# frasermince/gym-cellular-automata

Hardware: AMD Instinct MI355X
Metric: cell-updates/sec, 4096x(256x256) ForestFireBulldozer (Alexandridis CA), per-GPU batch (higher is better)
Workload: dtype u8 cells / i16 ages / f32 probabilities

## Files before the change

gym-cellular-automata_amd/csrc/gca_alex_march.hip:

```cpp
#include "gca_alex_rule.h"

#include <type_traits>

#ifndef GCA_MARCH_FLAT_OCC
#define GCA_MARCH_FLAT_OCC 4
#endif
#ifndef GCA_MARCH_OBS_FLAT_OCC
#define GCA_MARCH_OBS_FLAT_OCC 3
#endif
#ifndef GCA_MARCH_XROW
#define GCA_MARCH_XROW 1
#endif

namespace {

constexpr int MW = 256;
constexpr int SH = 16;

struct MarchObs {
    const float4* col;
    const int32_t* night;
    float* rgb;
    const int32_t* action;
    int action_stride, n_choices;
    uint32_t mode_bits;
    uint8_t* refit;
};
constexpr uint32_t OBS_GRID = 0u, OBS_ZERO = 1u, OBS_NONE = 2u;
constexpr uint32_t OBS_CHK_GRID = 4u, OBS_CHK_BLUR = 8u;

__device__ __forceinline__ uint32_t from_prev(uint32_t v) {
    return (uint32_t)__builtin_amdgcn_mov_dpp((int)v, 0x138, 0xF, 0xF, true);
}
__device__ __forceinline__ uint32_t from_next(uint32_t v) {
    return (uint32_t)__builtin_amdgcn_mov_dpp((int)v, 0x130, 0xF, 0xF, true);
}
__device__ __forceinline__ uint32_t from_prev_or(uint32_t old, uint32_t v) {
    return (uint32_t)__builtin_amdgcn_update_dpp((int)old, (int)v, 0x138, 0xF, 0xF, false);
}
__device__ __forceinline__ uint32_t from_next_or(uint32_t old, uint32_t v) {
    return (uint32_t)__builtin_amdgcn_update_dpp((int)old, (int)v, 0x130, 0xF, 0xF, false);
}

template <int J> __device__ __forceinline__ uint64_t byte_lanes(uint32_t x) {
    static_assert(J >= 0 && J < 4, "byte 0..3");
    uint64_t m;
    const uint32_t zero = 0u;
    if constexpr (J == 0) asm("v_cmp_ne_u32_sdwa %0, %1, %2 src0_sel:BYTE_0 src1_sel:DWORD" : "=s"(m) : "v"(x), "s"(zero));
    if constexpr (J == 1) asm("v_cmp_ne_u32_sdwa %0, %1, %2 src0_sel:BYTE_1 src1_sel:DWORD" : "=s"(m) : "v"(x), "s"(zero));
    if constexpr (J == 2) asm("v_cmp_ne_u32_sdwa %0, %1, %2 src0_sel:BYTE_2 src1_sel:DWORD" : "=s"(m) : "v"(x), "s"(zero));
    if constexpr (J == 3) asm("v_cmp_ne_u32_sdwa %0, %1, %2 src0_sel:BYTE_3 src1_sel:DWORD" : "=s"(m) : "v"(x), "s"(zero));
    return m;
}
__device__ __forceinline__ uint32_t lanes_select(uint32_t c, uint64_t m) {
    uint32_t o;
    asm("v_cndmask_b32_e64 %0, 0, %1, %2" : "=v"(o) : "v"(c), "s"(m));
    return o;
}

__host__ __device__ constexpr uint32_t win_mask(int o, int j, int k) {
    uint32_t m = 0;
    for (int b = 0; b < 4; ++b) {
        const int c = 4 * o + b - j;
        if (c >= -k && c <= k) m |= 1u << (8 * b);
    }
    return m;
}
__host__ __device__ constexpr bool win_full(int o, int j, int k) { return j - k <= 4 * o && 4 * o + 3 <= j + k; }
template <bool HALO = false>
__device__ __forceinline__ void window4(uint32_t X, int k, uint32_t (&B)[4], uint32_t z = 0u, uint32_t h1 = 0u,
                                        uint32_t h2 = 0u) {
    uint32_t n[5] = {0u, 0u, X, 0u, 0u};
    if (k >= 1) {
        n[1] = HALO ? from_prev_or(h1, X) : from_prev(X);
        n[3] = HALO ? from_next_or(h1, X) : from_next(X);
    }
    if (k >= 5) {
        n[0] = HALO ? from_prev_or(h2, n[1]) : from_prev(n[1]);
        n[4] = HALO ? from_next_or(h2, n[3]) : from_next(n[3]);
    }
    constexpr uint32_t ONES = 0x01010101u;
    bool use0 = false, useL = false, useR = false, useLR = false;
#pragma unroll
    for (int j = 0; j < 4; ++j) {
        const bool f0 = win_full(0, j, k), fl = win_full(-1, j, k), fr = win_full(1, j, k);
        if (f0 && fl && fr) useLR = true;
        else if (f0 && fl) useL = true;
        else if (f0 && fr) useR = true;
        else if (f0) use0 = true;
    }
    uint32_t S0 = 0u, SL = 0u, SR = 0u, SLR = 0u;
    if (use0 || useL || useR || useLR) S0 = __builtin_amdgcn_udot4(n[2], ONES, z, false);
    if (useL || useLR) SL = __builtin_amdgcn_udot4(n[1], ONES, S0, false);
    if (useR) SR = __builtin_amdgcn_udot4(n[3], ONES, S0, false);
    if (useLR) SLR = __builtin_amdgcn_udot4(n[3], ONES, SL, false);
#pragma unroll
    for (int j = 0; j < 4; ++j) {
        const bool f0 = win_full(0, j, k), fl = win_full(-1, j, k), fr = win_full(1, j, k);
        const bool run = f0;
        uint32_t acc = !run ? z : (fl && fr) ? SLR : fl ? SL : fr ? SR : S0;
#pragma unroll
        for (int o = -2; o <= 2; ++o) {
            if (run && (o == 0 || (o == -1 && fl) || (o == 1 && fr))) continue;
            const uint32_t m = win_mask(o, j, k);
            if (m) acc = __builtin_amdgcn_udot4(n[o + 2], m, acc, false);
        }
        B[j] = acc;
    }
}

__device__ __forceinline__ float4 ldf4(const float* p) { return *reinterpret_cast<const float4*>(p); }
__device__ __forceinline__ gca_f2 m_recip(float v0, float v1) {
    const gca_f2 x = {v0, v1};
    const gca_f2 r0 = {__builtin_amdgcn_rcpf(v0), __builtin_amdgcn_rcpf(v1)};
    const gca_f2 ee = __builtin_elementwise_fma(-x, r0, (gca_f2){1.0f, 1.0f});
    return __builtin_elementwise_fma(ee, r0, r0);
}
__device__ __forceinline__ void m_edge_both(float v0, float v1, gca_f2& own, gca_f2& nb) {
    const gca_f2 rc = m_recip(v0, v1);
    asm("v_max_f32_e64 %0, %1, -%2" : "=v"(own.x) : "v"(v0), "v"(rc.x));
    asm("v_max_f32_e64 %0, %1, -%2" : "=v"(own.y) : "v"(v1), "v"(rc.y));
    asm("v_max_f32_e64 %0, -%1, %2" : "=v"(nb.x) : "v"(v0), "v"(rc.x));
    asm("v_max_f32_e64 %0, -%1, %2" : "=v"(nb.y) : "v"(v1), "v"(rc.y));
}
__device__ __forceinline__ void m_edge_both4(const float4& v, gca_f2& oa, gca_f2& na, gca_f2& ob, gca_f2& nb) {
    const gca_f2 x0 = {v.x, v.y}, x1 = {v.z, v.w};
    const gca_f2 r0 = {__builtin_amdgcn_rcpf(v.x), __builtin_amdgcn_rcpf(v.y)};
    const gca_f2 r1 = {__builtin_amdgcn_rcpf(v.z), __builtin_amdgcn_rcpf(v.w)};
    const gca_f2 e0 = __builtin_elementwise_fma(-x0, r0, (gca_f2){1.0f, 1.0f});
    const gca_f2 e1 = __builtin_elementwise_fma(-x1, r1, (gca_f2){1.0f, 1.0f});
    const gca_f2 c0 = __builtin_elementwise_fma(e0, r0, r0);
    const gca_f2 c1 = __builtin_elementwise_fma(e1, r1, r1);
    asm("v_max_f32_e64 %0, %1, -%2" : "=v"(oa.x) : "v"(v.x), "v"(c0.x));
    asm("v_max_f32_e64 %0, %1, -%2" : "=v"(oa.y) : "v"(v.y), "v"(c0.y));
    asm("v_max_f32_e64 %0, %1, -%2" : "=v"(ob.x) : "v"(v.z), "v"(c1.x));
    asm("v_max_f32_e64 %0, %1, -%2" : "=v"(ob.y) : "v"(v.w), "v"(c1.y));
    asm("v_max_f32_e64 %0, -%1, %2" : "=v"(na.x) : "v"(v.x), "v"(c0.x));
    asm("v_max_f32_e64 %0, -%1, %2" : "=v"(na.y) : "v"(v.y), "v"(c0.y));
    asm("v_max_f32_e64 %0, -%1, %2" : "=v"(nb.x) : "v"(v.z), "v"(c1.x));
    asm("v_max_f32_e64 %0, -%1, %2" : "=v"(nb.y) : "v"(v.w), "v"(c1.y));
}
__device__ __forceinline__ void m_edge_own4(const float4& v, gca_f2& oa, gca_f2& ob) {
    const gca_f2 x0 = {v.x, v.y}, x1 = {v.z, v.w};
    const gca_f2 r0 = {__builtin_amdgcn_rcpf(v.x), __builtin_amdgcn_rcpf(v.y)};
    const gca_f2 r1 = {__builtin_amdgcn_rcpf(v.z), __builtin_amdgcn_rcpf(v.w)};
    const gca_f2 e0 = __builtin_elementwise_fma(-x0, r0, (gca_f2){1.0f, 1.0f});
    const gca_f2 e1 = __builtin_elementwise_fma(-x1, r1, (gca_f2){1.0f, 1.0f});
    const gca_f2 c0 = __builtin_elementwise_fma(e0, r0, r0);
    const gca_f2 c1 = __builtin_elementwise_fma(e1, r1, r1);
    asm("v_max_f32_e64 %0, %1, -%2" : "=v"(oa.x) : "v"(v.x), "v"(c0.x));
    asm("v_max_f32_e64 %0, %1, -%2" : "=v"(oa.y) : "v"(v.y), "v"(c0.y));
    asm("v_max_f32_e64 %0, %1, -%2" : "=v"(ob.x) : "v"(v.z), "v"(c1.x));
    asm("v_max_f32_e64 %0, %1, -%2" : "=v"(ob.y) : "v"(v.w), "v"(c1.y));
}
template <class T, class B> __device__ __forceinline__ T ld_at(const B* base, uint32_t off) {
    return *reinterpret_cast<const T*>(reinterpret_cast<const unsigned char*>(base) + off);
}
template <class T, class B> __device__ __forceinline__ T ld_nt(const B* base, uint32_t off) {
    constexpr int N = (int)(sizeof(T) / 4);
    typedef uint32_t vt __attribute__((ext_vector_type(N)));
    typedef const __attribute__((address_space(1))) unsigned char gbyte;
    typedef const __attribute__((address_space(1))) vt gvt;
    const vt v = __builtin_nontemporal_load((gvt*)((gbyte*)base + off));
    return __builtin_bit_cast(T, v);
}
constexpr uint32_t WZ = 0x4B000000u;
__device__ __forceinline__ gca_f2 wsum_f2(uint32_t b0, uint32_t b1) {
    return (gca_f2){__uint_as_float(b0), __uint_as_float(b1)} - (gca_f2){8388608.0f, 8388608.0f};
}
typedef uint16_t u16x2 __attribute__((ext_vector_type(2)));
typedef int16_t i16x2 __attribute__((ext_vector_type(2)));
__device__ __forceinline__ i16x2 bitcast_i16x2(uint32_t v) { return __builtin_bit_cast(i16x2, v); }
__device__ __forceinline__ u16x2 bitcast_u16x2(uint32_t v) { return __builtin_bit_cast(u16x2, v); }
template <class T> __device__ __forceinline__ uint32_t bitcast_u32(T v) { return __builtin_bit_cast(uint32_t, v); }

constexpr int XI = 16;
constexpr int XS_ONE = 13, XS_TWO = 14;

template <int R, bool OBS, bool GROW, int NSEG, int FLATM>
__global__ __launch_bounds__(NSEG == 1 ? 256 : 64 * NSEG) __attribute__((amdgpu_waves_per_eu(OBS ? (FLATM ? GCA_MARCH_OBS_FLAT_OCC : 2) : (FLATM ? GCA_MARCH_FLAT_OCC : 3), OBS ? (FLATM ? GCA_MARCH_OBS_FLAT_OCC : 2) : (FLATM ? GCA_MARCH_FLAT_OCC : 3)))) void alex_march_kernel(
    gca_alex_params p, int H, int nwaves, const uint8_t* __restrict__ grid_in, uint8_t* __restrict__ grid_out,
    const int16_t* age_in, int16_t* age_out,
    const uint8_t* __restrict__ vd, const uint16_t* __restrict__ dbits, const float* __restrict__ es,
    const int32_t* __restrict__ wind_index, const uint32_t* __restrict__ rng_step, int32_t* __restrict__ counts,
    const uint8_t* __restrict__ act_in, uint8_t* __restrict__ act_out, MarchObs obs) {
    constexpr int NF = 2 * R + 1;
    constexpr int RB = R;
    constexpr bool HALO = NSEG > 1;
    constexpr bool SMASK = !HALO && !OBS && FLATM >= 1;
    constexpr int WPB = HALO ? NSEG : 4;
    constexpr int W = MW * NSEG;
    __shared__ float lut[WPB][16];
    __shared__ float4 colw[WPB][8];
    __shared__ float4 img[OBS ? WPB : 1][OBS ? 192 : 1];
    __shared__ uint32_t fring[WPB][2 * NF * 64];
    __shared__ uint32_t xch[HALO ? 2 : 1][HALO ? NSEG + 2 : 1][4][HALO ? XI : 1];
    __shared__ uint32_t qfl[HALO ? NSEG : 1];
    constexpr bool FLAT = FLATM >= 1, UNI = FLATM == 2;
    constexpr bool XROW = GCA_MARCH_XROW && !HALO && OBS && !FLAT;
    __shared__ float4 xrow[XROW ? 4 : 1][3][XROW ? 64 : 1];
    __shared__ uint32_t xok[XROW ? 4 : 1];

    const int tid = threadIdx.x, wl = __builtin_amdgcn_readfirstlane(tid >> 6), lane = tid & 63;
    const int nb = (int)gridDim.x;
    const int xcd = (int)blockIdx.x & 7, slot = (int)blockIdx.x >> 3;
    const int qn8 = nb >> 3, rn8 = nb & 7;
    const int lb = (xcd < rn8 ? xcd * (qn8 + 1) : rn8 * (qn8 + 1) + (xcd - rn8) * qn8) + slot;
    int strips, e, s, g;
    if constexpr (!HALO) {
        const int wv = lb * 4 + wl;
        if (wv >= nwaves) {
            if constexpr (XROW) {
                if (lane == 0) xok[wl] = 0u;
                __builtin_amdgcn_fence(__ATOMIC_RELEASE, "workgroup", "local");
                __builtin_amdgcn_s_barrier();
            }
            return;
        }
        strips = H / SH;
        e = wv / strips;
        s = wv - e * strips;
        g = 0;
    } else {
        if (lb * NSEG >= nwaves) return;
        strips = H / SH;
        e = lb / strips;
        s = lb - e * strips;
        g = wl;
    }
    const int s0 = s * SH;
    const uint32_t HW = (uint32_t)H * W;
    const uint8_t* gE = grid_in + (size_t)e * HW;
    uint8_t* gO = grid_out + (size_t)e * HW;
    const int16_t* aE = age_in + (size_t)e * HW;
    int16_t* aO = age_out + (size_t)e * HW;
    const uint8_t* vE = UNI ? vd : vd + (size_t)e * HW;
    const uint16_t* dE = dbits + (size_t)e * (HW >> 4);
    const float* sE = FLAT ? es : es + (size_t)e * 4 * HW;
    const uint32_t lc = HALO ? (uint32_t)(MW * g) + 4u * (uint32_t)lane : 4u * (uint32_t)lane;
    const uint32_t ld16 = HALO ? lc >> 4 : (uint32_t)(lane >> 2);
    const uint32_t lane_a = 2u * lc, lane_s = 4u * lc, lane_d = 2u * ld16;
    const uint32_t Fp = rep4((uint32_t)p.fire), Ep = rep4((uint32_t)p.empty), Tp = rep4((uint32_t)p.tree);

    if (lane < 16) lut[wl][lane] = gca_alex_lut_entry(p, lane);
    if (OBS && lane < 6) colw[wl][lane] = obs.col[6 * (obs.night[e] != 0 ? 1 : 0) + lane];
    uint32_t omode = 0u;
    if constexpr (OBS && !HALO) {
        if (obs.action) {
            const int choice = min(max(obs.action[(size_t)e * obs.action_stride + 2], 0), obs.n_choices - 1);
            omode = (uint32_t)__builtin_amdgcn_readfirstlane((int)((obs.mode_bits >> (4 * choice)) & 0xFu));
        }
    }
    auto row0_refit = [&](uint32_t x0, uint32_t x1) -> uint8_t {
        const uint32_t odd = ((x0 + 0x7D7D7D7Du) | x0 | (x1 + 0x7D7D7D7Du) | x1) & 0x80808080u;
        bool pos = false;
        if (omode & OBS_CHK_GRID) pos |= __ballot(x0 != 0u) != 0ull;
        if (omode & OBS_CHK_BLUR) {
            auto hsum = [&](uint32_t x) {
                uint32_t L = __builtin_amdgcn_alignbyte(x, from_prev(x), 3);
                uint32_t Rt = __builtin_amdgcn_alignbyte(from_next(x), x, 1);
                if (lane == 0) L = (x << 8) | (x & 0xFFu);
                if (lane == 63) Rt = (x >> 8) | (x & 0xFF000000u);
                return L + x + Rt;
            };
            const uint32_t S = 2u * hsum(x0) + hsum(x1);
            pos |= __ballot(((S + 0x7B7B7B7Bu) & 0x80808080u) != 0u) != 0ull;
        }
        const bool bad = __ballot(odd != 0u) != 0ull;
        return ((omode & 3u) == OBS_NONE || bad || ((omode & (OBS_CHK_GRID | OBS_CHK_BLUR)) && !pos)) ? 1 : 0;
    };
    __builtin_amdgcn_fence(__ATOMIC_RELEASE, "wavefront");
    __builtin_amdgcn_wave_barrier();
    __builtin_amdgcn_fence(__ATOMIC_ACQUIRE, "wavefront");

    auto graw = [&](int r) -> uint32_t {
        return (r >= 0 && r < H) ? *reinterpret_cast<const uint32_t*>(gE + (uint32_t)r * W + lc) : Ep;
    };
    auto draw_bits = [&](int r) -> uint32_t {
        return (r >= 0 && r < H) ? (uint32_t)dE[(uint32_t)r * (W / 16) + ld16] : 0u;
    };
    auto dflags = [&](uint32_t w16) -> uint32_t { return gca_spread4(w16 >> (4 * (lane & 3))); };
    auto write_rgb_row = [&](int r, uint32_t tB, uint32_t fB, uint32_t dfl) {
        if constexpr (OBS) {
            if ((omode & 3u) == OBS_NONE) return;
            if ((omode & 3u) == OBS_ZERO) tB = fB = 0u;
            const uint32_t kidx = 2u * gca_spread4(tB) + 4u * gca_spread4(fB) + (dfl & 0x01010101u);
            float* im = reinterpret_cast<float*>(img[wl]) + 12 * lane;
#pragma unroll
            for (int j = 0; j < 4; ++j) {
                const float4 c = colw[wl][(kidx >> (8 * j)) & 0xFFu];
                im[3 * j + 0] = c.x;
                im[3 * j + 1] = c.y;
                im[3 * j + 2] = c.z;
            }
            __builtin_amdgcn_fence(__ATOMIC_RELEASE, "wavefront");
            __builtin_amdgcn_wave_barrier();
            __builtin_amdgcn_fence(__ATOMIC_ACQUIRE, "wavefront");
            typedef float f4t __attribute__((ext_vector_type(4)));
            float* row = obs.rgb + ((size_t)e * H + r) * (W * 3) + (HALO ? (size_t)(MW * 3) * g : 0);
            float4 v[3];
#pragma unroll
            for (int t = 0; t < 3; ++t) v[t] = img[wl][64 * t + lane];
#pragma unroll
            for (int t = 0; t < 3; ++t)
                __builtin_nontemporal_store((f4t){v[t].x, v[t].y, v[t].z, v[t].w},
                                            reinterpret_cast<f4t*>(row + 4 * (64 * t + lane)));
            __builtin_amdgcn_fence(__ATOMIC_RELEASE, "wavefront");
            __builtin_amdgcn_wave_barrier();
            __builtin_amdgcn_fence(__ATOMIC_ACQUIRE, "wavefront");
        }
    };

    auto xrow_publish = [&](bool ok, const float4* planes) {
        if constexpr (XROW) {
            if (ok) {
#pragma unroll
                for (int k = 0; k < 3; ++k) xrow[wl][k][lane] = planes[k];
            }
            if (lane == 0) xok[wl] = ok ? 1u : 0u;
            __builtin_amdgcn_fence(__ATOMIC_RELEASE, "workgroup", "local");
            __builtin_amdgcn_s_barrier();
            __builtin_amdgcn_fence(__ATOMIC_ACQUIRE, "workgroup", "local");
        }
    };

    uint32_t g_init[NF - 1];
#pragma unroll
    for (int t = 0; t < NF - 1; ++t) g_init[t] = graw(s0 - RB + t);
    auto quiet_copy = [&](auto row) {
        int cE = 0, cT = 0;
#pragma unroll
        for (int i = 0; i < SH; ++i) {
            const int r = s0 + i;
            const uint32_t o = (uint32_t)r * W + lc;
            const uint32_t gw = row(i);
            __builtin_nontemporal_store(gw, reinterpret_cast<uint32_t*>(gO + o));
            if (age_in != age_out) *reinterpret_cast<uint2*>(aO + o) = *reinterpret_cast<const uint2*>(aE + o);
            cE += __builtin_popcount(bytes_eq01(gw, Ep));
            cT += __builtin_popcount(bytes_eq01(gw, Tp));
            if (OBS) write_rgb_row(r, gca_eq_nib(gw, Tp), 0u, dflags(draw_bits(r)));
        }
        if constexpr (OBS && !HALO) {
            if (obs.refit && s0 == 0) {
                const uint8_t rf = row0_refit(row(0), row(1));
                if (lane == 0) obs.refit[e] = rf;
            }
        }
        if (act_out && lane == 0) act_out[((size_t)e * strips + s) * NSEG + g] = 0;
        if (counts) {
#pragma unroll
            for (int off = 32; off > 0; off >>= 1) {
                cE += __shfl_xor(cE, off);
                cT += __shfl_xor(cT, off);
            }
            if (lane == 0) {
                if (cE) atomicAdd(counts + 3 * e + 0, cE);
                if (cT) atomicAdd(counts + 3 * e + 1, cT);
            }
        }
    };
    bool quiet = false;
    if (!HALO && act_out && act_in) {
        const uint8_t* A = act_in + (size_t)e * strips;
        quiet = !(A[s] | (s > 0 ? A[s - 1] : 0) | (s + 1 < strips ? A[s + 1] : 0));
    } else if constexpr (!GROW) {
        auto has_fire = [&](uint32_t x) {
            const uint32_t v = x ^ Fp;
            return (v - 0x01010101u) & ~v & 0x80808080u;
        };
        if (__ballot((has_fire(g_init[RB - 1]) | has_fire(g_init[RB])) != 0u) == 0ull) {
            uint32_t gq[SH];
            gq[0] = g_init[RB];
            uint32_t f = has_fire(graw(s0 + SH));
#pragma unroll
            for (int i = 1; i < SH; ++i) {
                gq[i] = graw(s0 + i);
                f |= has_fire(gq[i]);
            }
            quiet = __ballot(f != 0u) == 0ull;
            if constexpr (!HALO) {
                if (quiet) {
                    xrow_publish(false, nullptr);
                    quiet_copy([&](int i) { return gq[i]; });
                    return;
                }
            }
        }
    }
    if constexpr (HALO) {
        if (wl == 0) {
#pragma unroll
            for (int j = 0; j < 4; ++j) {
                const int idx = 4 * lane + j;
                const int item = idx & 15, li = (idx >> 4) & 3, sl = ((idx >> 6) & 1) ? NSEG + 1 : 0, pa = idx >> 7;
                xch[pa][sl][li][item] = (item == XS_ONE || item == XS_TWO) ? 0x3F800000u : 0u;
            }
        }
        if (lane == 0) qfl[wl] = quiet ? 1u : 0u;
        __builtin_amdgcn_fence(__ATOMIC_RELEASE, "workgroup", "local");
        __builtin_amdgcn_s_barrier();
        __builtin_amdgcn_fence(__ATOMIC_ACQUIRE, "workgroup", "local");
        uint32_t all = 1u;
#pragma unroll
        for (int w = 0; w < NSEG; ++w) all &= qfl[w];
        quiet = all != 0u;
    }
    if (quiet) {
        xrow_publish(false, nullptr);
        quiet_copy([&](int i) { return *reinterpret_cast<const uint32_t*>(gE + (uint32_t)(s0 + i) * W + lc); });
        return;
    }

    uint32_t* FR = fring[wl];
    auto ring_put = [&](int t, uint32_t v) {
        const int sl = (2 * NF - 2 - t) % NF;
        FR[sl * 64 + lane] = v;
        FR[(sl + NF) * 64 + lane] = v;
    };
#pragma unroll
    for (int t = 0; t < NF - 1; ++t) ring_put(t, bytes_eq01(g_init[t], Fp));
    constexpr int DB = 2, ND = DB + 3;
    uint32_t dring[ND];
#pragma unroll
    for (int t = 0; t < ND - 1; ++t) dring[t] = dflags(draw_bits(s0 - DB + t));
    uint32_t nG = graw(s0 + R), nD = draw_bits(s0 + 2), nOwn = graw(s0);
    uint32_t nVD = UNI ? 0u : *reinterpret_cast<const uint32_t*>(vE + (size_t)s0 * W + lc);
    uint2 nAge = *reinterpret_cast<const uint2*>(aE + (size_t)s0 * W + lc);
    float4 sc[4], sn[4];
#pragma unroll
    for (int k = 0; k < 4; ++k) {
        if constexpr (FLAT) {
            sc[k] = sn[k] = make_float4(1.0f, 1.0f, 1.0f, 1.0f);
        } else {
            sc[k] = ldf4(sE + (size_t)k * HW + (size_t)s0 * W + lc);
            sn[k] = ldf4(sE + (size_t)k * HW + (size_t)min(s0 + 1, H - 1) * W + lc);
        }
    }
    __builtin_amdgcn_fence(__ATOMIC_RELEASE, "wavefront");
    __builtin_amdgcn_wave_barrier();
    __builtin_amdgcn_fence(__ATOMIC_ACQUIRE, "wavefront");
    xrow_publish(true, sc);
    const bool xuse = XROW && wl < 3 && s0 + SH < H && xok[XROW ? wl + 1 : 0] != 0u;
    uint32_t V[R + 1] = {};
    uint32_t Dv1 = 0u, Dv2 = 0u;

    const bool col_lo = lane == 0 && (!HALO || g == 0), col_hi = lane == 63 && (!HALO || g == NSEG - 1);
    const uint32_t xo1 = HALO ? (lane == 63 ? (uint32_t)(((g + 2) * 4 + 0) * XI) : (uint32_t)((g * 4 + 3) * XI)) : 0u;
    const uint32_t xo2 = HALO ? (lane == 63 ? (uint32_t)(((g + 2) * 4 + 1) * XI) : (uint32_t)((g * 4 + 2) * XI)) : 0u;
    auto prep_own = [&](float4& v) {
        gca_f2 a, b;
        m_edge_own4(v, a, b);
        v = make_float4(col_lo ? 1.0f : a.x, a.y, b.x, col_hi ? 1.0f : b.y);
    };
    if constexpr (!FLAT) {
#pragma unroll
        for (int k = 0; k < 3; ++k) prep_own(sc[k]);
    }

    constexpr int NHW = (R + 2) / 2;
    gca_f2 windp[4], hdwp[NHW];
    {
        const int widx = wind_index[e];
#pragma unroll
        for (int q = 0; q < 4; ++q) {
            const int d0 = 2 * q, d1 = 2 * q + 1;
            windp[q] = (gca_f2){p.winds[widx][d0 < 4 ? d0 : d0 + 1], p.winds[widx][d1 < 4 ? d1 : d1 + 1]};
            asm volatile("" : "+v"(windp[q]));
        }
#pragma unroll
        for (int q = 0; q < NHW; ++q) {
            hdwp[q] = (gca_f2){p.heat_dw[2 * q], 2 * q + 1 <= R ? p.heat_dw[2 * q + 1] : 0.0f};
            asm volatile("" : "+v"(hdwp[q]));
        }
    }
    gca_f2 avd = {1.0f, 1.0f};
    if constexpr (UNI) {
        const int b = p.vd_uniform & 0xFF;
        avd = (gca_f2){gca_alex_lut_entry(p, b & 7), gca_alex_lut_entry(p, 8 + ((b >> 4) & 7))};
        asm volatile("" : "+v"(avd));
    }
    auto bcast = [](gca_f2 v, int h) -> gca_f2 {
        return h ? __builtin_shufflevector(v, v, 1, 1) : __builtin_shufflevector(v, v, 0, 0);
    };
    const uint32_t step = rng_step ? rng_step[e] : 0u;
    const uint32_t k0 = (uint32_t)p.seed, k1 = (uint32_t)(p.seed >> 32);
    const uint32_t env_id = (uint32_t)(p.env_offset + e);
    constexpr uint32_t PM0 = 0xD2511F53u, PM1 = 0xCD9E8D57u, PW0 = 0x9E3779B9u, PW1 = 0xBB67AE85u;
    const uint64_t pq1 = (uint64_t)PM1 * step;
    const uint32_t pu0 = (uint32_t)(pq1 >> 32) ^ env_id ^ k0;
    const uint64_t pq2 = (uint64_t)PM0 * pu0;
    const uint32_t pkc = (uint32_t)GCA_TAG_ALEX_CELL ^ k1;
    const uint32_t pkc_age = (uint32_t)GCA_TAG_ALEX_AGE ^ k1;
    const uint32_t pka = (uint32_t)pq1 ^ (k0 + PW0);
    const uint32_t pkb = (uint32_t)(pq2 >> 32) ^ (k1 + PW1);
    const uint32_t pl2 = (uint32_t)pq2;
    auto philox_cell = [&](uint32_t x0, uint32_t rk0, uint32_t rk1, uint32_t ktag) -> u32x4 {
        const uint64_t p0 = (uint64_t)PM0 * x0;
        const uint32_t hi0 = (uint32_t)(p0 >> 32), lo0 = (uint32_t)p0;
        const uint64_t p1 = (uint64_t)PM1 * (hi0 ^ ktag);
        u32x4 c = u32x4{(uint32_t)(p1 >> 32) ^ pka, (uint32_t)p1, lo0 ^ pkb, pl2};
#pragma unroll
        for (int i = 2; i < 10; ++i) {
            const uint64_t a = (uint64_t)PM0 * c.x;
            const uint64_t b = (uint64_t)PM1 * c.z;
            const uint32_t n0 = __builtin_amdgcn_bitop3_b32((uint32_t)(b >> 32), c.y, rk0 + (uint32_t)i * PW0, 0x96);
            const uint32_t n2 = __builtin_amdgcn_bitop3_b32((uint32_t)(a >> 32), c.w, rk1 + (uint32_t)i * PW1, 0x96);
            c = u32x4{n0, (uint32_t)b, n2, (uint32_t)a};
        }
        return c;
    };
    const float pt24 = __fmul_rn(p.p_tree, 16777216.0f);
    const float w_in_minus_bd = __fsub_rn(p.dous_inner, p.dous_border);
    const uint32_t codes = (p.empty & 0xFFu) | ((p.tree & 0xFFu) << 8) | ((p.fire & 0xFFu) << 16);
    int cntE = 0, cntT = 0, cntF = 0;
    uint64_t mP[4] = {}, mC[4] = {};
    if constexpr (SMASK) {
        const uint32_t fa = bytes_eq01(g_init[RB - 1], Fp), fb = bytes_eq01(g_init[RB], Fp);
        mP[0] = byte_lanes<0>(fa); mP[1] = byte_lanes<1>(fa); mP[2] = byte_lanes<2>(fa); mP[3] = byte_lanes<3>(fa);
        mC[0] = byte_lanes<0>(fb); mC[1] = byte_lanes<1>(fb); mC[2] = byte_lanes<2>(fb); mC[3] = byte_lanes<3>(fb);
    }
    uint32_t out_row0 = 0u;

    auto row = [&](const int i, float4 (&SC)[4], float4 (&SN)[4], auto parity) {
        const int r = s0 + i;
        const uint32_t gnew = nG, dnew = nD, own = nOwn, vdw = nVD;
        const uint2 agep = nAge;
        {
            const int rg = r + 1 + R, rd = r + 3;
            const uint32_t r1 = (uint32_t)min(r + 1, H - 1);
            const uint32_t gl = ld_at<uint32_t>(gE + (size_t)min(rg, H - 1) * W, lc);
            const uint32_t d = ld_at<uint16_t>(dE + (size_t)min(rd, H - 1) * (W / 16), lane_d);
            nOwn = ld_at<uint32_t>(gE + (size_t)r1 * W, lc);
            if constexpr (!UNI) nVD = ld_nt<uint32_t>(vE + (size_t)r1 * W, lc);
            nAge = ld_nt<uint2>(aE + (size_t)r1 * W, lane_a);
            nG = rg < H ? gl : Ep;
            nD = rd < H ? d : 0u;
        }
        bool need_next = i + 1 < SH;
        auto load_next_slopes = [&]() {
            if constexpr (XROW) {
                if (i == SH - 2 && xuse) {
#pragma unroll
                    for (int k = 0; k < 3; ++k) SC[k] = xrow[wl + 1][k][lane];
                    SC[3] = SC[2];
                    return;
                }
            }
            const bool need3 = need_next && i + 2 < SH;
            const float* sb = need_next ? sE : es;
            const float* sb3 = need3 ? sE : es;
            const uint32_t rs = need_next ? (uint32_t)min(r + 2, H - 1) : 0u;
            const uint32_t rs3 = need3 ? rs : 0u;
#pragma unroll
            for (int k = 0; k < 4; ++k)
                SC[k] = ld_nt<float4>((k == 3 ? sb3 : sb) + (size_t)k * HW + (size_t)(k == 3 ? rs3 : rs) * W, lane_s);
        };
        uint32_t* Fb = FR + (NF - 1 - (uint32_t)i % NF) * 64;
        {
            const uint32_t fnew = bytes_eq01(gnew, Fp);
            Fb[lane] = fnew;
            Fb[NF * 64 + lane] = fnew;
        }
        __builtin_amdgcn_fence(__ATOMIC_RELEASE, "wavefront");
        __builtin_amdgcn_wave_barrier();
        __builtin_amdgcn_fence(__ATOMIC_ACQUIRE, "wavefront");
        uint32_t fm1, f0, fp1;
        {
            uint32_t rw[NF];
#pragma unroll
            for (int t = 0; t < NF; ++t) rw[t] = Fb[(NF - 1 - t) * 64 + lane];
            V[1] = rw[RB - 1] + rw[RB] + rw[RB + 1];
#pragma unroll
            for (int k = 2; k <= R; ++k) V[k] = V[k - 1] + rw[RB + k] + rw[RB - k];
            fm1 = rw[RB - 1];
            f0 = rw[RB];
            fp1 = rw[RB + 1];
            if constexpr (R >= 3)
                need_next = need_next && __ballot((rw[RB] | rw[RB + 1] | rw[RB + 2] | rw[RB + 3]) != 0u) != 0ull;
        }
        dring[ND - 1] = dflags(dnew);
        Dv1 = dring[1] + dring[2] + dring[3];
        Dv2 = Dv1 + dring[0] + dring[4];
        uint64_t mN[4] = {};
        auto next_lanes = [&]() {
            if constexpr (SMASK) {
                mN[0] = byte_lanes<0>(fp1);
                mN[1] = byte_lanes<1>(fp1);
                mN[2] = byte_lanes<2>(fp1);
                mN[3] = byte_lanes<3>(fp1);
            }
        };

        const uint32_t* xr = nullptr;
        const uint32_t* xr2 = nullptr;
        uint32_t hfm1 = 0u, hf0 = 0u, hfp1 = 0u;
        if constexpr (HALO) {
            constexpr int PAR = decltype(parity)::value;
            if (lane < 2 || lane >= 62) {
                const int xl = lane < 2 ? lane : lane - 60;
                uint4* xd = reinterpret_cast<uint4*>(&xch[PAR][g + 1][xl][0]);
                uint32_t vv[8];
#pragma unroll
                for (int k = 0; k < 8; ++k) vv[k] = k + 1 <= R ? V[k + 1] : 0u;
                const uint32_t sA = lane < 32 ? __float_as_uint(SC[3].x) : __float_as_uint(SN[2].w);
                xd[0] = make_uint4(vv[0], vv[1], vv[2], vv[3]);
                xd[1] = make_uint4(vv[4], vv[5], vv[6], vv[7]);
                xd[2] = make_uint4(Dv1, Dv2, fm1, f0);
                xd[3] = make_uint4(fp1, sA, __float_as_uint(SN[0].x), 0u);
            }
            __builtin_amdgcn_fence(__ATOMIC_RELEASE, "workgroup", "local");
            __builtin_amdgcn_s_barrier();
            __builtin_amdgcn_fence(__ATOMIC_ACQUIRE, "workgroup", "local");
            xr = &xch[PAR][0][0][0] + xo1;
            xr2 = &xch[PAR][0][0][0] + xo2;
            hfm1 = xr[10];
            hf0 = xr[11];
            hfp1 = xr[12];
        }

        const uint32_t treeB = gca_eq_nib(own, Tp), emptyB = gca_eq_nib(own, Ep);
        auto shl_c = [](uint32_t x, uint32_t h) {
            return __builtin_amdgcn_alignbyte(x, HALO ? from_prev_or(h, x) : from_prev(x), 3);
        };
        auto shr_c = [](uint32_t x, uint32_t h) {
            return __builtin_amdgcn_alignbyte(HALO ? from_next_or(h, x) : from_next(x), x, 1);
        };
        auto dir_mask = [&](int d) -> uint32_t {
            const uint32_t row = d < 3 ? fm1 : (d < 5 ? f0 : fp1);
            const uint32_t hrow = d < 3 ? hfm1 : (d < 5 ? hf0 : hfp1);
            const int dc = d < 3 ? d - 1 : (d == 3 ? -1 : (d == 4 ? 1 : d - 6));
            uint32_t m = dc < 0 ? shl_c(row, hrow) : (dc > 0 ? shr_c(row, hrow) : row);
            m *= 0xFFu;
            asm volatile("" : "+v"(m));
            return m;
        };
        auto dir_lanes = [&](int d, int j) -> uint64_t {
            const uint64_t* m = d < 3 ? mP : (d < 5 ? mC : mN);
            const int dc = d < 3 ? d - 1 : (d == 3 ? -1 : (d == 4 ? 1 : d - 6));
            if (dc < 0) return j > 0 ? m[j - 1] : m[3] << 1;
            if (dc > 0) return j < 3 ? m[j + 1] : m[0] >> 1;
            return m[j];
        };
        const uint32_t fireB = (f0 * 0x01020408u) >> 24;
        const uint32_t vor = fm1 | f0 | fp1, hvor = hfm1 | hf0 | hfp1;
        const uint32_t anyfire = (((vor | shl_c(vor, hvor) | shr_c(vor, hvor)) & 0x01010101u) * 0x01020408u) >> 24;
        gca_f2 qn[2] = {{1.0f, 1.0f}, {1.0f, 1.0f}};
        const bool row_need = __ballot((treeB & anyfire) != 0u) != 0ull;
        const bool kill_row = r == 0 || r == H - 1;
        const bool kill_next = r + 1 == H - 1;
        auto prep_next = [&](int k, bool want_nb, float (&nbv)[4]) {
            gca_f2 oa, ob, na, nb2;
            if (want_nb) {
                m_edge_both4(SN[k], oa, na, ob, nb2);
                nbv[0] = na.x; nbv[1] = na.y; nbv[2] = nb2.x; nbv[3] = nb2.y;
            } else {
                m_edge_own4(SN[k], oa, ob);
            }
            SN[k] = make_float4(col_lo ? 1.0f : oa.x, oa.y, ob.x, col_hi ? 1.0f : ob.y);
        };
        if (!row_need) {
            next_lanes();
            if constexpr (!FLAT) {
                load_next_slopes();
                float unused[4];
#pragma unroll
                for (int k = 0; k < 3; ++k) prep_next(k, false, unused);
            }
        } else {
            gca_f2 ph[2] = {{p.heat0, p.heat0}, {p.heat0, p.heat0}};
#pragma unroll
            for (int k = 0; k <= R; ++k) {
                uint32_t B[4];
                if (k == 0) {
#pragma unroll
                    for (int j = 0; j < 4; ++j) B[j] = (f0 >> (8 * j)) & 0xFFu;
                } else {
                    if constexpr (HALO)
                        window4<true>(V[k], k, B, WZ, xr[k - 1], k >= 5 ? xr2[k - 1] : 0u);
                    else
                        window4(V[k], k, B, WZ);
                }
                gca_f2 bs[2];
#pragma unroll
                for (int h = 0; h < 2; ++h)
                    bs[h] = k == 0 ? (gca_f2){(float)B[2 * h], (float)B[2 * h + 1]} : wsum_f2(B[2 * h], B[2 * h + 1]);
#pragma unroll
                for (int h = 0; h < 2; ++h) ph[h] = __builtin_elementwise_fma(bcast(hdwp[k >> 1], k & 1), bs[h], ph[h]);
                asm volatile("" : "+v"(ph[0]), "+v"(ph[1]));
                __builtin_amdgcn_sched_barrier(0);
            }
            const bool dous_any = __ballot((Dv2 | (HALO ? xr[8] | xr[9] : 0u)) != 0u) != 0ull;
            if (dous_any) {
                uint32_t D1[4], D2[4];
                if constexpr (HALO) {
                    window4<true>(Dv1, 1, D1, WZ, xr[8]);
                    window4<true>(Dv2, 2, D2, WZ, xr[9]);
                } else {
                    window4(Dv1, 1, D1, WZ);
                    window4(Dv2, 2, D2, WZ);
                }
                gca_f2 d1[2], d2[2], dz[2];
#pragma unroll
                for (int h = 0; h < 2; ++h) d1[h] = wsum_f2(D1[2 * h], D1[2 * h + 1]);
#pragma unroll
                for (int h = 0; h < 2; ++h) d2[h] = wsum_f2(D2[2 * h], D2[2 * h + 1]);
#pragma unroll
                for (int h = 0; h < 2; ++h) dz[h] = (gca_f2){w_in_minus_bd, w_in_minus_bd} * d1[h];
#pragma unroll
                for (int h = 0; h < 2; ++h)
                    dz[h] = __builtin_elementwise_fma((gca_f2){p.dous_border, p.dous_border}, d2[h], dz[h]);
#pragma unroll
                for (int h = 0; h < 2; ++h) ph[h] = ph[h] - dz[h];
            }
            if constexpr (UNI) {
#pragma unroll
                for (int h = 0; h < 2; ++h) ph[h] = ph[h] * bcast(avd, 0);
#pragma unroll
                for (int h = 0; h < 2; ++h) ph[h] = ph[h] * bcast(avd, 1);
            } else {
                gca_f2 av[2], ad[2];
#pragma unroll
                for (int h = 0; h < 2; ++h) {
                    const uint32_t b0 = (vdw >> (16 * h)) & 0xFFu, b1 = (vdw >> (16 * h + 8)) & 0xFFu;
                    av[h] = (gca_f2){lut[wl][b0 & 7u], lut[wl][b1 & 7u]};
                    ad[h] = (gca_f2){lut[wl][8 + (b0 >> 4)], lut[wl][8 + (b1 >> 4)]};
                }
#pragma unroll
                for (int h = 0; h < 2; ++h) ph[h] = ph[h] * av[h];
#pragma unroll
                for (int h = 0; h < 2; ++h) ph[h] = ph[h] * ad[h];
            }
            auto dir_pass = [&](auto kill_tag) {
                constexpr bool KILL = decltype(kill_tag)::value;
                auto apply = [&](int d, const float (&a)[4]) {
                    asm volatile("" : "+v"(ph[0]), "+v"(ph[1]), "+v"(qn[0]), "+v"(qn[1]));
                    const gca_f2 wd2 = bcast(windp[d >> 1], d & 1);
                    gca_f2 c[2];
                    if constexpr (KILL) {
#pragma unroll
                        for (int h = 0; h < 2; ++h) c[h] = gca_pk_mul_clamp01(ph[h], wd2);
                    } else {
                        gca_f2 t[2];
#pragma unroll
                        for (int h = 0; h < 2; ++h) t[h] = ph[h] * wd2;
#pragma unroll
                        for (int h = 0; h < 2; ++h) c[h] = gca_pk_mul_clamp01(t[h], (gca_f2){a[2 * h], a[2 * h + 1]});
                    }
                    uint32_t cm[2][2];
                    if constexpr (SMASK) {
#pragma unroll
                        for (int h = 0; h < 2; ++h) {
                            cm[h][0] = lanes_select(__float_as_uint(c[h].x), dir_lanes(d, 2 * h));
                            cm[h][1] = lanes_select(__float_as_uint(c[h].y), dir_lanes(d, 2 * h + 1));
                        }
                    } else {
                        const uint32_t Md = dir_mask(d);
#pragma unroll
                        for (int h = 0; h < 2; ++h) {
                            cm[h][0] = __float_as_uint(c[h].x) & (uint32_t)(int32_t)(int8_t)(Md >> (16 * h));
                            cm[h][1] = __float_as_uint(c[h].y) & (uint32_t)(int32_t)(int8_t)(Md >> (16 * h + 8));
                        }
                    }
#pragma unroll
                    for (int h = 0; h < 2; ++h)
                        qn[h] = __builtin_elementwise_fma(-qn[h], (gca_f2){__uint_as_float(cm[h][0]), __uint_as_float(cm[h][1])},
                                                          qn[h]);
                    __builtin_amdgcn_sched_barrier(0);
                };
                const float one[4] = {1.0f, 1.0f, 1.0f, 1.0f};
                uint32_t h45 = 0x3F800000u, h7 = 0x3F800000u;
                if constexpr (HALO && !KILL) {
                    gca_f2 o_, n_;
                    m_edge_both(__uint_as_float(xr[XS_ONE]), __uint_as_float(xr[XS_TWO]), o_, n_);
                    h45 = __float_as_uint(n_.x);
                    h7 = __float_as_uint(n_.y);
                }
#pragma unroll
                for (int d = 0; d < 3; ++d) {
                    const float a[4] = {SC[d].x, SC[d].y, SC[d].z, SC[d].w};
                    apply(d, KILL ? one : a);
                }
                if (KILL) {
                    apply(3, one);
                    apply(4, one);
                } else {
                    gca_f2 oa, ob, na, nb2;
                    m_edge_both4(SC[3], oa, na, ob, nb2);
                    const float a3[4] = {col_lo ? 1.0f : oa.x, oa.y, ob.x, col_hi ? 1.0f : ob.y};
                    apply(3, a3);
                    const float nx = __uint_as_float((uint32_t)__builtin_amdgcn_update_dpp(
                        (int)h45, (int)__float_as_uint(na.x), 0x130, 0xF, 0xF, false));
                    const float a4[4] = {col_lo ? 1.0f : na.y, nb2.x, nb2.y, nx};
                    apply(4, a4);
                }
                if constexpr (!FLAT) load_next_slopes();
                next_lanes();
                float nb[4];
                if constexpr (!FLAT) prep_next(2, !KILL, nb);
                if (KILL) {
                    apply(5, one);
                } else {
                    const float pv = __uint_as_float((uint32_t)__builtin_amdgcn_update_dpp(
                        (int)h45, (int)__float_as_uint(nb[3]), 0x138, 0xF, 0xF, false));
                    const float a5[4] = {pv, nb[0], nb[1], col_hi ? 1.0f : nb[2]};
                    apply(5, a5);
                }
                if constexpr (!FLAT) prep_next(1, !KILL, nb);
                if (KILL) {
                    apply(6, one);
                } else {
                    const float a6[4] = {col_lo ? 1.0f : nb[0], nb[1], nb[2], col_hi ? 1.0f : nb[3]};
                    apply(6, a6);
                }
                if constexpr (!FLAT) prep_next(0, !KILL, nb);
                if (KILL) {
                    apply(7, one);
                } else {
                    const float nx = __uint_as_float((uint32_t)__builtin_amdgcn_update_dpp(
                        (int)h7, (int)__float_as_uint(nb[0]), 0x130, 0xF, 0xF, false));
                    const float a7[4] = {col_lo ? 1.0f : nb[1], nb[2], nb[3], nx};
                    apply(7, a7);
                }
            };
            if (FLAT || kill_row)
                dir_pass(std::true_type{});
            else
                dir_pass(std::false_type{});
        }
        if (kill_next) {
#pragma unroll
            for (int k = 0; k < 3; ++k) SN[k] = make_float4(1.0f, 1.0f, 1.0f, 1.0f);
        }

        const uint32_t needB = (treeB & anyfire) | (GROW ? emptyB : 0u);
        const uint32_t lin0 = (uint32_t)r * W + lc;
        uint32_t burn = 0u, grow = 0u, NA[2];
        const bool wave_draws = __ballot(needB != 0u) != 0ull;
        uint32_t rk0 = k0, rk1 = k1;
        asm volatile("" : "+s"(rk0), "+s"(rk1));
        u32x4 X = u32x4{0u, 0u, 0u, 0u};
        if (wave_draws) X = philox_cell(lin0 >> 2, rk0, rk1, pkc);
        const uint32_t xw[4] = {X.x, X.y, X.z, X.w};
#pragma unroll
        for (int h = 0; h < 2; ++h) {
            const gca_f2 thr = __builtin_elementwise_fma(qn[h], (gca_f2){-16777216.0f, -16777216.0f},
                                                         (gca_f2){16777216.0f, 16777216.0f});
            const float u0 = (float)(xw[2 * h] >> 8), u1 = (float)(xw[2 * h + 1] >> 8);
            burn |= (u0 < thr.x ? 1u : 0u) << (2 * h);
            burn |= (u1 < thr.y ? 1u : 0u) << (2 * h + 1);
            if constexpr (GROW) {
                grow |= (u0 < pt24 ? 1u : 0u) << (2 * h);
                grow |= (u1 < pt24 ? 1u : 0u) << (2 * h + 1);
            }
        }
        burn &= treeB;
        grow &= emptyB;
        {
            const uint32_t spare = __builtin_amdgcn_perm(__builtin_amdgcn_perm(X.w, X.z, 0x0c0c0400u),
                                                         __builtin_amdgcn_perm(X.y, X.x, 0x0c0c0400u), 0x05040100u);
            const uint32_t n0 = (uint32_t)randint_ms(spare, p.age_lo, p.age_hi);
            NA[0] = NA[1] = __builtin_amdgcn_perm(n0, n0, 0x05040100u);
            if (__ballot((burn & (burn - 1u)) != 0u) != 0ull) {
                const u32x4 Y = philox_cell(lin0 >> 2, rk0, rk1, pkc_age);
                const uint32_t nk[4] = {n0, (uint32_t)randint_ms(Y.x, p.age_lo, p.age_hi),
                                        (uint32_t)randint_ms(Y.y, p.age_lo, p.age_hi),
                                        (uint32_t)randint_ms(Y.z, p.age_lo, p.age_hi)};
                uint32_t a[4];
#pragma unroll
                for (int j = 0; j < 4; ++j) {
                    const uint32_t rank = (uint32_t)__builtin_popcount(burn & ((1u << j) - 1u));
                    a[j] = rank == 0 ? nk[0] : (rank == 1 ? nk[1] : (rank == 2 ? nk[2] : nk[3]));
                }
                NA[0] = __builtin_amdgcn_perm(a[1], a[0], 0x05040100u);
                NA[1] = __builtin_amdgcn_perm(a[3], a[2], 0x05040100u);
            }
        }

        const uint32_t agw[2] = {agep.x, agep.y};
        uint32_t le1;
        if (!p.burnout_eq1) {
            const uint32_t y0 = bitcast_u32(__builtin_elementwise_sub_sat(bitcast_i16x2(agw[0]), (i16x2){2, 2}));
            const uint32_t y1 = bitcast_u32(__builtin_elementwise_sub_sat(bitcast_i16x2(agw[1]), (i16x2){2, 2}));
            le1 = ((y0 >> 15) & 1u) | ((y0 >> 30) & 2u) | ((y1 >> 13) & 4u) | ((y1 >> 28) & 8u);
        } else {
            le1 = 0u;
#pragma unroll
            for (int j = 0; j < 4; ++j)
                le1 |= ((int32_t)(int16_t)(agw[j >> 1] >> (16 * (j & 1))) == 1) ? (1u << j) : 0u;
        }
        const uint32_t newF = burn | (fireB & ~le1);
        const uint32_t newT = (treeB & ~burn) | grow;
        const uint32_t newE = (emptyB & ~grow) | (fireB & le1);
        const uint32_t keepB = ~(treeB | emptyB | fireB) & 0xFu;
        uint32_t sel = gca_spread4(newT) + 2u * gca_spread4(newF);
        sel |= (gca_spread4(keepB) * 0xFFu) & 0x07060504u;
        const uint32_t outw = __builtin_amdgcn_perm(own, codes, sel);
        uint32_t nag[2];
#pragma unroll
        for (int h = 0; h < 2; ++h) {
            const uint32_t fh = ((fireB >> (2 * h)) & 1u) | (((fireB >> (2 * h + 1)) & 1u) << 16);
            const uint32_t a1 = bitcast_u32(bitcast_u16x2(agw[h]) - bitcast_u16x2(fh));
            const uint32_t bm = (((burn >> (2 * h)) & 1u) * 0xFFFFu) | (((burn >> (2 * h + 1)) & 1u) * 0xFFFF0000u);
            nag[h] = gca_bfi32(bm, NA[h], a1);
        }
        const size_t o = (size_t)r * W + lc;
        __builtin_nontemporal_store(outw, reinterpret_cast<uint32_t*>(gO + o));
        { typedef uint32_t u2v __attribute__((ext_vector_type(2)));
          __builtin_nontemporal_store((u2v){nag[0], nag[1]}, reinterpret_cast<u2v*>(aO + o)); }
        write_rgb_row(r, newT, newF, dring[DB]);
        if constexpr (OBS && !HALO) {
            if (obs.refit && r < 2) {
                if (r == 0) {
                    out_row0 = outw;
                } else {
                    const uint8_t rf = row0_refit(out_row0, outw);
                    if (lane == 0) obs.refit[e] = rf;
                }
            }
        }
        cntT += __builtin_popcount(newT);
        cntF += __builtin_popcount(newF);
        cntE += __builtin_popcount(newE);

#pragma unroll
        for (int t = 0; t < ND - 1; ++t) dring[t] = dring[t + 1];
        if constexpr (SMASK) {
#pragma unroll
            for (int j = 0; j < 4; ++j) {
                mP[j] = mC[j];
                mC[j] = mN[j];
            }
        }
    };
#pragma unroll 1
    for (int i = 0; i < SH; i += 2) {
        row(i, sc, sn, std::integral_constant<int, 0>{});
        row(i + 1, sn, sc, std::integral_constant<int, 1>{});
    }

    if (counts || act_out) {
        const bool anyF = __ballot(cntF != 0) != 0ull;
        if (act_out && lane == 0) act_out[((size_t)e * strips + s) * NSEG + g] = anyF ? 1 : 0;
        if (counts) {
#pragma unroll
            for (int off = 32; off > 0; off >>= 1) {
                cntT += __shfl_xor(cntT, off);
                cntF += __shfl_xor(cntF, off);
                cntE += __shfl_xor(cntE, off);
            }
            if (lane == 0) {
                if (cntE) atomicAdd(counts + 3 * e + 0, cntE);
                if (cntT) atomicAdd(counts + 3 * e + 1, cntT);
                if (cntF) atomicAdd(counts + 3 * e + 2, cntF);
            }
        }
    }
}

template <int R, bool OBS, bool GROW, int NSEG, int FLATM>
void launch_march_n(const gca_alex_params& p, int E, int H, const uint8_t* gi, uint8_t* go, const int16_t* ai,
                    int16_t* ao, const uint8_t* vd, const uint16_t* db, const float* es, const int32_t* wi,
                    const uint32_t* rs, int32_t* counts, const uint8_t* act_in, uint8_t* act_out, MarchObs obs,
                    hipStream_t st) {
    const int nwaves = E * (H / SH) * NSEG;
    if constexpr (NSEG == 1)
        hipLaunchKernelGGL((alex_march_kernel<R, OBS, GROW, 1, FLATM>), dim3((unsigned)((nwaves + 3) / 4)), dim3(256), 0, st, p,
                           H, nwaves, gi, go, ai, ao, vd, db, es, wi, rs, counts, act_in, act_out, obs);
    else
        hipLaunchKernelGGL((alex_march_kernel<R, OBS, GROW, NSEG, FLATM>), dim3((unsigned)(nwaves / NSEG)), dim3(64 * NSEG), 0,
                           st, p, H, nwaves, gi, go, ai, ao, vd, db, es, wi, rs, counts, act_in, act_out, obs);
}
template <int R, bool OBS, bool GROW, int FLATM>
void launch_march_g(const gca_alex_params& p, int E, int H, int W, const uint8_t* gi, uint8_t* go, const int16_t* ai,
                    int16_t* ao, const uint8_t* vd, const uint16_t* db, const float* es, const int32_t* wi,
                    const uint32_t* rs, int32_t* counts, const uint8_t* act_in, uint8_t* act_out, MarchObs obs,
                    hipStream_t st) {
    if (W == MW)
        launch_march_n<R, OBS, GROW, 1, FLATM>(p, E, H, gi, go, ai, ao, vd, db, es, wi, rs, counts, act_in, act_out, obs, st);
    else if (W == 2 * MW)
        launch_march_n<R, OBS, GROW, 2, FLATM>(p, E, H, gi, go, ai, ao, vd, db, es, wi, rs, counts, act_in, act_out, obs, st);
    else
        launch_march_n<R, OBS, GROW, 4, FLATM>(p, E, H, gi, go, ai, ao, vd, db, es, wi, rs, counts, act_in, act_out, obs, st);
}
template <int R, bool OBS>
void launch_march(const gca_alex_params& p, int E, int H, int W, const uint8_t* gi, uint8_t* go, const int16_t* ai,
                  int16_t* ao, const uint8_t* vd, const uint16_t* db, const float* es, const int32_t* wi,
                  const uint32_t* rs, int32_t* counts, const uint8_t* act_in, uint8_t* act_out, MarchObs obs,
                  hipStream_t st) {
    const bool grow = p.p_tree > 0.0f;
    const int fm = es ? 0 : (vd ? 1 : 2);
#define GCA_MARCH_FM(FM)                                                                                                \
    if (grow)                                                                                                         \
        launch_march_g<R, OBS, true, FM>(p, E, H, W, gi, go, ai, ao, vd, db, es, wi, rs, counts, act_in, act_out, obs, st); \
    else                                                                                                              \
        launch_march_g<R, OBS, false, FM>(p, E, H, W, gi, go, ai, ao, vd, db, es, wi, rs, counts, act_in, act_out, obs, st);
    if (fm == 0) {
        GCA_MARCH_FM(0)
    } else if (fm == 1) {
// ... 134 lines not shown
```

Measured before the change: 1242 billion.

## Skip center heat term, use coarse wave-need test, and exec-masked FMA chain

Several micro-optimizations go into the SMASK march path. The k=0 (center cell) heat term is skipped when the parameters show it contributes nothing. The per-lane anyfire computation is replaced by a coarser wave-level ballot (any fire and any tree in the wave). Per-direction mask-select plus product accumulation is replaced by an inline-asm chain that sets the EXEC mask and issues v_fma_f32 only on active lanes. A disabled-by-default option defers dous flag decoding until needed. Risks: the coarser need test means more rows take the expensive path. Also, needB still reads anyfire, which is now zero under WNEED, so burn masking may rely only on the treeB mask. The exec-writing asm may interfere with compiler scheduling or correctness.

```diff
diff --git a/gym-cellular-automata_amd/csrc/gca_alex_march.hip b/gym-cellular-automata_amd/csrc/gca_alex_march.hip
--- a/gym-cellular-automata_amd/csrc/gca_alex_march.hip
+++ b/gym-cellular-automata_amd/csrc/gca_alex_march.hip
@@ -10,6 +10,19 @@
 #endif
 #ifndef GCA_MARCH_XROW
 #define GCA_MARCH_XROW 1
+#endif
+
+#ifndef GCA_MARCH_SKIP_K0
+#define GCA_MARCH_SKIP_K0 1
+#endif
+#ifndef GCA_MARCH_WAVE_NEED
+#define GCA_MARCH_WAVE_NEED 1
+#endif
+#ifndef GCA_MARCH_DOUS_WORDS
+#define GCA_MARCH_DOUS_WORDS 0
+#endif
+#ifndef GCA_MARCH_EXEC_CHAIN
+#define GCA_MARCH_EXEC_CHAIN 1
 #endif
 
 namespace {
@@ -56,6 +69,21 @@
     uint32_t o;
     asm("v_cndmask_b32_e64 %0, 0, %1, %2" : "=v"(o) : "v"(c), "s"(m));
     return o;
+}
+
+__device__ __forceinline__ void lanes_fma_chain(float (&q)[4], uint64_t m0, uint64_t m1, uint64_t m2, uint64_t m3,
+                                                float c0, float c1, float c2, float c3) {
+    asm("s_mov_b64 exec, %4\n\t"
+        "v_fma_f32 %0, -%0, %8, %0\n\t"
+        "s_mov_b64 exec, %5\n\t"
+        "v_fma_f32 %1, -%1, %9, %1\n\t"
+        "s_mov_b64 exec, %6\n\t"
+        "v_fma_f32 %2, -%2, %10, %2\n\t"
+        "s_mov_b64 exec, %7\n\t"
+        "v_fma_f32 %3, -%3, %11, %3\n\t"
+        "s_mov_b64 exec, -1"
+        : "+v"(q[0]), "+v"(q[1]), "+v"(q[2]), "+v"(q[3])
+        : "s"(m0), "s"(m1), "s"(m2), "s"(m3), "v"(c0), "v"(c1), "v"(c2), "v"(c3));
 }
 
 __host__ __device__ constexpr uint32_t win_mask(int o, int j, int k) {
@@ -188,6 +216,9 @@
     constexpr int RB = R;
     constexpr bool HALO = NSEG > 1;
     constexpr bool SMASK = !HALO && !OBS && FLATM >= 1;
+    constexpr bool XCHAIN = GCA_MARCH_EXEC_CHAIN && SMASK;
+    constexpr bool WNEED = GCA_MARCH_WAVE_NEED && SMASK;
+    constexpr bool DWORDS = GCA_MARCH_DOUS_WORDS && !HALO && !OBS;
     constexpr int WPB = HALO ? NSEG : 4;
     constexpr int W = MW * NSEG;
     __shared__ float lut[WPB][16];
@@ -422,7 +453,7 @@
     constexpr int DB = 2, ND = DB + 3;
     uint32_t dring[ND];
 #pragma unroll
-    for (int t = 0; t < ND - 1; ++t) dring[t] = dflags(draw_bits(s0 - DB + t));
+    for (int t = 0; t < ND - 1; ++t) dring[t] = DWORDS ? draw_bits(s0 - DB + t) : dflags(draw_bits(s0 - DB + t));
     uint32_t nG = graw(s0 + R), nD = draw_bits(s0 + 2), nOwn = graw(s0);
     uint32_t nVD = UNI ? 0u : *reinterpret_cast<const uint32_t*>(vE + (size_t)s0 * W + lc);
     uint2 nAge = *reinterpret_cast<const uint2*>(aE + (size_t)s0 * W + lc);
@@ -513,6 +544,8 @@
     const float w_in_minus_bd = __fsub_rn(p.dous_inner, p.dous_border);
     const uint32_t codes = (p.empty & 0xFFu) | ((p.tree & 0xFFu) << 8) | ((p.fire & 0xFFu) << 16);
     int cntE = 0, cntT = 0, cntF = 0;
+    const bool skip_k0 = GCA_MARCH_SKIP_K0 && (__float_as_uint(p.heat_dw[0]) & 0x7F800000u) != 0x7F800000u &&
+                         ((uint32_t)p.tree & 0xFFu) != ((uint32_t)p.fire & 0xFFu);
     uint64_t mP[4] = {}, mC[4] = {};
     if constexpr (SMASK) {
         const uint32_t fa = bytes_eq01(g_init[RB - 1], Fp), fb = bytes_eq01(g_init[RB], Fp);
@@ -578,9 +611,13 @@
             if constexpr (R >= 3)
                 need_next = need_next && __ballot((rw[RB] | rw[RB + 1] | rw[RB + 2] | rw[RB + 3]) != 0u) != 0ull;
         }
-        dring[ND - 1] = dflags(dnew);
-        Dv1 = dring[1] + dring[2] + dring[3];
-        Dv2 = Dv1 + dring[0] + dring[4];
+        if constexpr (DWORDS) {
+            dring[ND - 1] = dnew;
+        } else {
+            dring[ND - 1] = dflags(dnew);
+            Dv1 = dring[1] + dring[2] + dring[3];
+            Dv2 = Dv1 + dring[0] + dring[4];
+        }
         uint64_t mN[4] = {};
         auto next_lanes = [&]() {
             if constexpr (SMASK) {
@@ -643,9 +680,16 @@
         };
         const uint32_t fireB = (f0 * 0x01020408u) >> 24;
         const uint32_t vor = fm1 | f0 | fp1, hvor = hfm1 | hf0 | hfp1;
-        const uint32_t anyfire = (((vor | shl_c(vor, hvor) | shr_c(vor, hvor)) & 0x01010101u) * 0x01020408u) >> 24;
         gca_f2 qn[2] = {{1.0f, 1.0f}, {1.0f, 1.0f}};
-        const bool row_need = __ballot((treeB & anyfire) != 0u) != 0ull;
+        float qs[4] = {1.0f, 1.0f, 1.0f, 1.0f};
+        uint32_t anyfire = 0u;
+        bool row_need;
+        if constexpr (WNEED) {
+            row_need = __ballot(vor != 0u) != 0ull && __ballot(treeB != 0u) != 0ull;
+        } else {
+            anyfire = (((vor | shl_c(vor, hvor) | shr_c(vor, hvor)) & 0x01010101u) * 0x01020408u) >> 24;
+            row_need = __ballot((treeB & anyfire) != 0u) != 0ull;
+        }
         const bool kill_row = r == 0 || r == H - 1;
         const bool kill_next = r + 1 == H - 1;
         auto prep_next = [&](int k, bool want_nb, float (&nbv)[4]) {
@@ -668,29 +712,39 @@
             }
         } else {
             gca_f2 ph[2] = {{p.heat0, p.heat0}, {p.heat0, p.heat0}};
-#pragma unroll
-            for (int k = 0; k <= R; ++k) {
+            if (!skip_k0) {
+                gca_f2 bs[2];
+#pragma unroll
+                for (int h = 0; h < 2; ++h)
+                    bs[h] = (gca_f2){(float)((f0 >> (16 * h)) & 0xFFu), (float)((f0 >> (16 * h + 8)) & 0xFFu)};
+#pragma unroll
+                for (int h = 0; h < 2; ++h) ph[h] = __builtin_elementwise_fma(bcast(hdwp[0], 0), bs[h], ph[h]);
+                asm volatile("" : "+v"(ph[0]), "+v"(ph[1]));
+                __builtin_amdgcn_sched_barrier(0);
+            }
+#pragma unroll
+            for (int k = 1; k <= R; ++k) {
                 uint32_t B[4];
-                if (k == 0) {
-#pragma unroll
-                    for (int j = 0; j < 4; ++j) B[j] = (f0 >> (8 * j)) & 0xFFu;
-                } else {
-                    if constexpr (HALO)
-                        window4<true>(V[k], k, B, WZ, xr[k - 1], k >= 5 ? xr2[k - 1] : 0u);
-                    else
-                        window4(V[k], k, B, WZ);
-                }
+                if constexpr (HALO)
+                    window4<true>(V[k], k, B, WZ, xr[k - 1], k >= 5 ? xr2[k - 1] : 0u);
+                else
+                    window4(V[k], k, B, WZ);
                 gca_f2 bs[2];
 #pragma unroll
-                for (int h = 0; h < 2; ++h)
-                    bs[h] = k == 0 ? (gca_f2){(float)B[2 * h], (float)B[2 * h + 1]} : wsum_f2(B[2 * h], B[2 * h + 1]);
+                for (int h = 0; h < 2; ++h) bs[h] = wsum_f2(B[2 * h], B[2 * h + 1]);
 #pragma unroll
                 for (int h = 0; h < 2; ++h) ph[h] = __builtin_elementwise_fma(bcast(hdwp[k >> 1], k & 1), bs[h], ph[h]);
                 asm volatile("" : "+v"(ph[0]), "+v"(ph[1]));
                 __builtin_amdgcn_sched_barrier(0);
             }
-            const bool dous_any = __ballot((Dv2 | (HALO ? xr[8] | xr[9] : 0u)) != 0u) != 0ull;
+            const bool dous_any =
+                DWORDS ? __ballot((dring[0] | dring[1] | dring[2] | dring[3] | dring[4]) != 0u) != 0ull
+                       : __ballot((Dv2 | (HALO ? xr[8] | xr[9] : 0u)) != 0u) != 0ull;
             if (dous_any) {
+                if constexpr (DWORDS) {
+                    Dv1 = dflags(dring[1]) + dflags(dring[2]) + dflags(dring[3]);
+                    Dv2 = Dv1 + dflags(dring[0]) + dflags(dring[4]);
+                }
                 uint32_t D1[4], D2[4];
                 if constexpr (HALO) {
                     window4<true>(Dv1, 1, D1, WZ, xr[8]);
@@ -733,7 +787,10 @@
             auto dir_pass = [&](auto kill_tag) {
                 constexpr bool KILL = decltype(kill_tag)::value;
                 auto apply = [&](int d, const float (&a)[4]) {
-                    asm volatile("" : "+v"(ph[0]), "+v"(ph[1]), "+v"(qn[0]), "+v"(qn[1]));
+                    if constexpr (XCHAIN)
+                        asm volatile("" : "+v"(ph[0]), "+v"(ph[1]), "+v"(qs[0]), "+v"(qs[1]), "+v"(qs[2]), "+v"(qs[3]));
+                    else
+                        asm volatile("" : "+v"(ph[0]), "+v"(ph[1]), "+v"(qn[0]), "+v"(qn[1]));
                     const gca_f2 wd2 = bcast(windp[d >> 1], d & 1);
                     gca_f2 c[2];
                     if constexpr (KILL) {
@@ -745,6 +802,12 @@
                         for (int h = 0; h < 2; ++h) t[h] = ph[h] * wd2;
 #pragma unroll
                         for (int h = 0; h < 2; ++h) c[h] = gca_pk_mul_clamp01(t[h], (gca_f2){a[2 * h], a[2 * h + 1]});
+                    }
+                    if constexpr (XCHAIN) {
+                        lanes_fma_chain(qs, dir_lanes(d, 0), dir_lanes(d, 1), dir_lanes(d, 2), dir_lanes(d, 3), c[0].x,
+                                        c[0].y, c[1].x, c[1].y);
+                        __builtin_amdgcn_sched_barrier(0);
+                        return;
                     }
                     uint32_t cm[2][2];
                     if constexpr (SMASK) {
@@ -835,7 +898,8 @@
         const uint32_t needB = (treeB & anyfire) | (GROW ? emptyB : 0u);
         const uint32_t lin0 = (uint32_t)r * W + lc;
         uint32_t burn = 0u, grow = 0u, NA[2];
-        const bool wave_draws = __ballot(needB != 0u) != 0ull;
+        const bool wave_draws =
+            WNEED ? row_need || (GROW && __ballot(emptyB != 0u) != 0ull) : __ballot(needB != 0u) != 0ull;
         uint32_t rk0 = k0, rk1 = k1;
         asm volatile("" : "+s"(rk0), "+s"(rk1));
         u32x4 X = u32x4{0u, 0u, 0u, 0u};
@@ -843,7 +907,8 @@
         const uint32_t xw[4] = {X.x, X.y, X.z, X.w};
 #pragma unroll
         for (int h = 0; h < 2; ++h) {
-            const gca_f2 thr = __builtin_elementwise_fma(qn[h], (gca_f2){-16777216.0f, -16777216.0f},
+            const gca_f2 qh = XCHAIN ? (gca_f2){qs[2 * h], qs[2 * h + 1]} : qn[h];
+            const gca_f2 thr = __builtin_elementwise_fma(qh, (gca_f2){-16777216.0f, -16777216.0f},
                                                          (gca_f2){16777216.0f, 16777216.0f});
             const float u0 = (float)(xw[2 * h] >> 8), u1 = (float)(xw[2 * h + 1] >> 8);
             burn |= (u0 < thr.x ? 1u : 0u) << (2 * h);
```

New measurement: 1227 billion. -1.2%, worse.
